# DarlingHang/st-nerf

Measured on NVIDIA H100. Metric: rays/sec, higher is better.
Workload: dtype f32 via fp16x3 split products (wgmma), f32 accumulate

## Files before the change

st-nerf_b200/csrc/mlp_tc.cu:

```cuda
#include <cuda_fp16.h>
#include <string.h>
#include <type_traits>
#include <vector>
#include "mlp_tc.cuh"
#include "resample.cuh"

namespace stnerf {

namespace {

constexpr int TILE_M = 128;
constexpr int ABLOCK = 16384;
constexpr int STAGE_BYTES = 16384;
constexpr int NTHREADS = 384;
constexpr int MATH_WG0 = 1, N_MATH_WARPS = 8;
constexpr int MAX_STAGE = 8;
constexpr int BAR_WFULL = 0, BAR_WEMPTY = 8, BAR_RAWFULL = 16, BAR_RAWEMPTY = 18;
constexpr int MISC_ROWS = 256;
constexpr int MISC_PART = MISC_ROWS + 128 * 24;
constexpr int MISC_CDF = MISC_PART + 2048;
constexpr int MISC_TOTAL = MISC_CDF + 512;

__device__ __forceinline__ uint32_t smem_u32(const void* p) { return (uint32_t)__cvta_generic_to_shared(p); }

__device__ __forceinline__ void mbar_init(uint32_t bar, uint32_t count) {
  asm volatile("mbarrier.init.shared::cta.b64 [%0], %1;" ::"r"(bar), "r"(count) : "memory");
}
__device__ __forceinline__ void mbar_arrive(uint32_t bar) {
  asm volatile("mbarrier.arrive.shared::cta.b64 _, [%0];" ::"r"(bar) : "memory");
}
__device__ __forceinline__ void mbar_arrive_if(uint32_t bar, bool pred) {
  asm volatile("{\n\t.reg .pred p;\n\tsetp.ne.b32 p, %1, 0;\n\t@p mbarrier.arrive.shared::cta.b64 _, [%0];\n\t}" ::"r"(bar), "r"((uint32_t)pred)
               : "memory");
}
__device__ __forceinline__ void mbar_expect_tx(uint32_t bar, uint32_t bytes) {
  asm volatile("mbarrier.arrive.expect_tx.shared::cta.b64 _, [%0], %1;" ::"r"(bar), "r"(bytes) : "memory");
}
__device__ __forceinline__ void mbar_wait(uint32_t bar, uint32_t parity) {
  asm volatile(
      "{\n\t.reg .pred p;\n\t.reg .u32 c;\n\t"
      "mov.u32 c, 0;\n"
      "WAIT_%=:\n\t"
      "mbarrier.try_wait.parity.shared::cta.b64 p, [%0], %1;\n\t"
      "@p bra.uni DONE_%=;\n\t"
      "add.u32 c, c, 1;\n\t"
      "setp.gt.u32 p, c, 67108864;\n\t"
      "@p trap;\n\t"
      "bra.uni WAIT_%=;\n"
      "DONE_%=:\n\t}" ::"r"(bar), "r"(parity)
      : "memory");
}
__device__ __forceinline__ void bulk_g2s(uint32_t dst, const void* src, uint32_t bytes, uint32_t bar) {
  asm volatile("cp.async.bulk.shared::cluster.global.mbarrier::complete_tx::bytes [%0], [%1], %2, [%3];" ::"r"(dst),
               "l"(src), "r"(bytes), "r"(bar)
               : "memory");
}
__device__ __forceinline__ void fence_proxy_async() { asm volatile("fence.proxy.async.shared::cta;" ::: "memory"); }
__device__ __forceinline__ void wg_bar_sync(int wg) { asm volatile("bar.sync %0, 128;" ::"r"(1 + wg) : "memory"); }

__device__ __forceinline__ void load_stage_elect(uint32_t dst, const void* src, uint32_t bytes, uint32_t bar) {
  asm volatile(
      "{\n\t.reg .pred pe;\n\t"
      "elect.sync _|pe, 0xffffffff;\n\t"
      "@pe mbarrier.arrive.expect_tx.shared::cta.b64 _, [%3], %2;\n\t"
      "@pe cp.async.bulk.shared::cluster.global.mbarrier::complete_tx::bytes [%0], [%1], %2, [%3];\n\t}" ::"r"(dst),
      "l"(src), "r"(bytes), "r"(bar)
      : "memory");
}

__device__ __forceinline__ uint64_t desc_sw128(uint32_t saddr) {
  return (uint64_t)((saddr >> 4) & 0x3FFF) | ((uint64_t)1 << 16) | ((uint64_t)(1024 >> 4) << 32) | ((uint64_t)1 << 62);
}
__device__ __forceinline__ uint64_t desc_sw64(uint32_t saddr) {
  return (uint64_t)((saddr >> 4) & 0x3FFF) | ((uint64_t)1 << 16) | ((uint64_t)(512 >> 4) << 32) | ((uint64_t)2 << 62);
}
__device__ __forceinline__ void wgmma_fence() { asm volatile("wgmma.fence.sync.aligned;" ::: "memory"); }
__device__ __forceinline__ void wgmma_commit() { asm volatile("wgmma.commit_group.sync.aligned;" ::: "memory"); }
template <int N>
__device__ __forceinline__ void wgmma_wait() { asm volatile("wgmma.wait_group.sync.aligned %0;" ::"n"(N) : "memory"); }
template <int R>
__device__ __forceinline__ void acc_fence(float (&d)[128]) {
#pragma unroll
  for (int i = 0; i < R; ++i) asm volatile("" : "+f"(d[i])::"memory");
}

__device__ __forceinline__ void wgmma_n256(float (&d)[128], uint64_t da, uint64_t db) {
  asm volatile(
      "{\n\t.reg .pred p;\n\tsetp.ne.b32 p, %130, 0;\n\t"
      "wgmma.mma_async.sync.aligned.m64n256k16.f32.f16.f16 "
      "{%0, %1, %2, %3, %4, %5, %6, %7, %8, %9, %10, %11, %12, %13, %14, %15, "
      "%16, %17, %18, %19, %20, %21, %22, %23, %24, %25, %26, %27, %28, %29, %30, %31, "
      "%32, %33, %34, %35, %36, %37, %38, %39, %40, %41, %42, %43, %44, %45, %46, %47, "
      "%48, %49, %50, %51, %52, %53, %54, %55, %56, %57, %58, %59, %60, %61, %62, %63, "
      "%64, %65, %66, %67, %68, %69, %70, %71, %72, %73, %74, %75, %76, %77, %78, %79, "
      "%80, %81, %82, %83, %84, %85, %86, %87, %88, %89, %90, %91, %92, %93, %94, %95, "
      "%96, %97, %98, %99, %100, %101, %102, %103, %104, %105, %106, %107, %108, %109, %110, %111, "
      "%112, %113, %114, %115, %116, %117, %118, %119, %120, %121, %122, %123, %124, %125, %126, %127}, "
      "%128, %129, p, 1, 1, 0, 0;\n\t}"
      : "+f"(d[0]), "+f"(d[1]), "+f"(d[2]), "+f"(d[3]), "+f"(d[4]), "+f"(d[5]), "+f"(d[6]), "+f"(d[7]),
        "+f"(d[8]), "+f"(d[9]), "+f"(d[10]), "+f"(d[11]), "+f"(d[12]), "+f"(d[13]), "+f"(d[14]), "+f"(d[15]),
        "+f"(d[16]), "+f"(d[17]), "+f"(d[18]), "+f"(d[19]), "+f"(d[20]), "+f"(d[21]), "+f"(d[22]), "+f"(d[23]),
        "+f"(d[24]), "+f"(d[25]), "+f"(d[26]), "+f"(d[27]), "+f"(d[28]), "+f"(d[29]), "+f"(d[30]), "+f"(d[31]),
        "+f"(d[32]), "+f"(d[33]), "+f"(d[34]), "+f"(d[35]), "+f"(d[36]), "+f"(d[37]), "+f"(d[38]), "+f"(d[39]),
        "+f"(d[40]), "+f"(d[41]), "+f"(d[42]), "+f"(d[43]), "+f"(d[44]), "+f"(d[45]), "+f"(d[46]), "+f"(d[47]),
        "+f"(d[48]), "+f"(d[49]), "+f"(d[50]), "+f"(d[51]), "+f"(d[52]), "+f"(d[53]), "+f"(d[54]), "+f"(d[55]),
        "+f"(d[56]), "+f"(d[57]), "+f"(d[58]), "+f"(d[59]), "+f"(d[60]), "+f"(d[61]), "+f"(d[62]), "+f"(d[63]),
        "+f"(d[64]), "+f"(d[65]), "+f"(d[66]), "+f"(d[67]), "+f"(d[68]), "+f"(d[69]), "+f"(d[70]), "+f"(d[71]),
        "+f"(d[72]), "+f"(d[73]), "+f"(d[74]), "+f"(d[75]), "+f"(d[76]), "+f"(d[77]), "+f"(d[78]), "+f"(d[79]),
        "+f"(d[80]), "+f"(d[81]), "+f"(d[82]), "+f"(d[83]), "+f"(d[84]), "+f"(d[85]), "+f"(d[86]), "+f"(d[87]),
        "+f"(d[88]), "+f"(d[89]), "+f"(d[90]), "+f"(d[91]), "+f"(d[92]), "+f"(d[93]), "+f"(d[94]), "+f"(d[95]),
        "+f"(d[96]), "+f"(d[97]), "+f"(d[98]), "+f"(d[99]), "+f"(d[100]), "+f"(d[101]), "+f"(d[102]), "+f"(d[103]),
        "+f"(d[104]), "+f"(d[105]), "+f"(d[106]), "+f"(d[107]), "+f"(d[108]), "+f"(d[109]), "+f"(d[110]), "+f"(d[111]),
        "+f"(d[112]), "+f"(d[113]), "+f"(d[114]), "+f"(d[115]), "+f"(d[116]), "+f"(d[117]), "+f"(d[118]), "+f"(d[119]),
        "+f"(d[120]), "+f"(d[121]), "+f"(d[122]), "+f"(d[123]), "+f"(d[124]), "+f"(d[125]), "+f"(d[126]), "+f"(d[127])
      : "l"(da), "l"(db), "r"(1));
}
__device__ __forceinline__ void wgmma_n128(float (&d)[128], uint64_t da, uint64_t db) {
  asm volatile(
      "{\n\t.reg .pred p;\n\tsetp.ne.b32 p, %66, 0;\n\t"
      "wgmma.mma_async.sync.aligned.m64n128k16.f32.f16.f16 "
      "{%0, %1, %2, %3, %4, %5, %6, %7, %8, %9, %10, %11, %12, %13, %14, %15, "
      "%16, %17, %18, %19, %20, %21, %22, %23, %24, %25, %26, %27, %28, %29, %30, %31, "
      "%32, %33, %34, %35, %36, %37, %38, %39, %40, %41, %42, %43, %44, %45, %46, %47, "
      "%48, %49, %50, %51, %52, %53, %54, %55, %56, %57, %58, %59, %60, %61, %62, %63}, "
      "%64, %65, p, 1, 1, 0, 0;\n\t}"
      : "+f"(d[0]), "+f"(d[1]), "+f"(d[2]), "+f"(d[3]), "+f"(d[4]), "+f"(d[5]), "+f"(d[6]), "+f"(d[7]),
        "+f"(d[8]), "+f"(d[9]), "+f"(d[10]), "+f"(d[11]), "+f"(d[12]), "+f"(d[13]), "+f"(d[14]), "+f"(d[15]),
        "+f"(d[16]), "+f"(d[17]), "+f"(d[18]), "+f"(d[19]), "+f"(d[20]), "+f"(d[21]), "+f"(d[22]), "+f"(d[23]),
        "+f"(d[24]), "+f"(d[25]), "+f"(d[26]), "+f"(d[27]), "+f"(d[28]), "+f"(d[29]), "+f"(d[30]), "+f"(d[31]),
        "+f"(d[32]), "+f"(d[33]), "+f"(d[34]), "+f"(d[35]), "+f"(d[36]), "+f"(d[37]), "+f"(d[38]), "+f"(d[39]),
        "+f"(d[40]), "+f"(d[41]), "+f"(d[42]), "+f"(d[43]), "+f"(d[44]), "+f"(d[45]), "+f"(d[46]), "+f"(d[47]),
        "+f"(d[48]), "+f"(d[49]), "+f"(d[50]), "+f"(d[51]), "+f"(d[52]), "+f"(d[53]), "+f"(d[54]), "+f"(d[55]),
        "+f"(d[56]), "+f"(d[57]), "+f"(d[58]), "+f"(d[59]), "+f"(d[60]), "+f"(d[61]), "+f"(d[62]), "+f"(d[63])
      : "l"(da), "l"(db), "r"(1));
}

template <int N>
__device__ __forceinline__ void wgmma_k16(float (&d)[128], uint64_t da, uint64_t db) {
  if (N == 256) wgmma_n256(d, da, db);
  else wgmma_n128(d, da, db);
}

__device__ __forceinline__ uint32_t pack_f16x2(float a, float b) {
  uint32_t r;
  asm("cvt.rn.satfinite.f16x2.f32 %0, %1, %2;" : "=r"(r) : "f"(b), "f"(a));
  return r;
}
__device__ __forceinline__ float2 unpack_f16x2(uint32_t p) {
  return __half22float2(*reinterpret_cast<const __half2*>(&p));
}

__host__ __device__ inline uint32_t sw128_offset(int row, int col) {
  return (uint32_t)((row >> 3) * 1024 + (row & 7) * 128 + ((((col >> 3) ^ (row & 7)) & 7) << 4) + ((col & 7) << 1));
}
__host__ __device__ inline uint32_t sw64_offset(int row, int col) {
  return (uint32_t)((row >> 3) * 512 + (row & 7) * 64 + ((((col >> 3) ^ ((row >> 1) & 3)) & 3) << 4) + ((col & 7) << 1));
}

enum { NET_SPACE = 0, NET_MOTION = 1 };

template <int NET> struct Sched;
template <> struct Sched<NET_SPACE> {
  static constexpr int N_LAYERS = 8;
  static constexpr int act_base = 0, enc_base = 8 * ABLOCK;
  static constexpr int LO_STRIDE = 4 * ABLOCK;
  static constexpr int ENC_LO_STRIDE = ABLOCK;
  static constexpr int n_stage = 3, stage_bytes = STAGE_BYTES;
  static constexpr int ring_base = 10 * ABLOCK, misc_base = ring_base + n_stage * stage_bytes, smem_total = misc_base + MISC_TOTAL;
  static_assert(smem_total <= 232448, "shared memory budget (227 KB per CTA)");
  __host__ __device__ static constexpr int n_out(int l) { return l == 7 ? 128 : 256; }
  __host__ __device__ static constexpr int act_chunks(int l) { return l == 0 ? 0 : 4; }
  __host__ __device__ static constexpr int enc_chunks(int l) { return (l == 0 || l == 4) ? 1 : 0; }
  __host__ __device__ static constexpr bool enc_first(int l) { return l == 4; }
};
template <> struct Sched<NET_MOTION> {
  static constexpr int N_LAYERS = 5;
  static constexpr int act_base = 0, enc_base = 0;
  static constexpr int LO_STRIDE = 2 * ABLOCK;
  static constexpr int ENC_LO_STRIDE = 2 * ABLOCK;
  static constexpr int n_stage = 8, stage_bytes = 8192;
  static constexpr int ring_base = 4 * ABLOCK, misc_base = ring_base + n_stage * stage_bytes, smem_total = misc_base + MISC_TOTAL;
  __host__ __device__ static constexpr int n_out(int) { return 128; }
  __host__ __device__ static constexpr int act_chunks(int l) { return l == 0 ? 0 : 2; }
  __host__ __device__ static constexpr int enc_chunks(int l) { return l == 0 ? 2 : 0; }
  __host__ __device__ static constexpr bool enc_first(int) { return false; }
};
static_assert(Sched<NET_SPACE>::n_stage <= MAX_STAGE && Sched<NET_MOTION>::n_stage <= MAX_STAGE, "barrier slots");

enum { A_HI = 0, A_LO = 1, A_HI_LO = 2 };
template <int A>
struct WStep {
  static constexpr int a = A;
  uint32_t offset;
  uint32_t sub;
};
template <int NET>
struct WSched {
  using S = Sched<NET>;
  __host__ __device__ static constexpr int n_chunks(int l) { return S::act_chunks(l) + S::enc_chunks(l); }
  __host__ __device__ static constexpr uint32_t stage_bytes(int l) { return (uint32_t)S::n_out(l) * 64; }
  __host__ __device__ static constexpr size_t layer_bytes(int l) { return (size_t)n_chunks(l) * 2  * 2  * stage_bytes(l); }
  __host__ __device__ static constexpr int chunk_at(int l, int c) {
    return S::enc_first(l) ? (c == 0 ? S::act_chunks(l) : c - 1) : c;
  }
  static constexpr bool enc_first_valid() {
    for (int l = 0; l < S::N_LAYERS; ++l)
      if (S::enc_first(l) && (S::act_chunks(l) == 0 || S::enc_chunks(l) == 0)) return false;
    return true;
  }
  static_assert(enc_first_valid(), "enc_first(l) needs activation chunks and an encoding chunk to reorder");
  template <bool LOFIRST, class C, class F>
  __device__ __forceinline__ static void for_each_step(int l, bool split, C&& chunk, F&& f) {
    const int nact = S::act_chunks(l), nch = nact + S::enc_chunks(l);
    const uint32_t bytes = stage_bytes(l);
    auto at = [&](const auto& a, int c, uint32_t sub, uint32_t lo_stage, auto op) {
      f(a, WStep<decltype(op)::value>{(2 * (2 * (uint32_t)c + sub) + lo_stage) * bytes, sub});
    };
    using HI = std::integral_constant<int, A_HI>;
    using LO = std::integral_constant<int, A_LO>;
    using HI_LO = std::integral_constant<int, A_HI_LO>;
    if (!LOFIRST || !split) {
      for (int c = 0; c < nch; ++c) {
        const auto a = chunk(chunk_at(l, c));
        for (uint32_t sub = 0; sub < 2; ++sub) {
          if (split) { at(a, c, sub, 1u, HI()); at(a, c, sub, 0u, HI_LO()); }
          else at(a, c, sub, 0u, HI());
        }
      }
    } else {
      for (int c = 0; c < nch; ++c) {
        const auto a = chunk(chunk_at(l, c));
        for (uint32_t sub = 0; sub < 2; ++sub) { at(a, c, sub, 1u, HI()); at(a, c, sub, 0u, LO()); }
      }
      for (int c = 0; c < nch; ++c) {
        const auto a = chunk(chunk_at(l, c));
        for (uint32_t sub = 0; sub < 2; ++sub) at(a, c, sub, 0u, HI());
      }
    }
  }
};

template <int NET>
__host__ __device__ constexpr size_t stream_bytes_per_tile() {
  size_t n = 0;
  for (int l = 0; l < Sched<NET>::N_LAYERS; ++l) n += WSched<NET>::layer_bytes(l);
  return n;
}

struct TcParams {
  FuseCoarse fuse;
  PointSrc src;
  const uint8_t* wstream;
  const float* aux;
  const float* cbuf;
  int exact;
  int single_last;
  int lo_first;
  float* raw;
  float* rgb_out;
// ... 145 lines not shown
        a = in4[d];
        if (lerp) {
          const float lo = d < 3 ? in4[d] : lo_t, hi = d < 3 ? in4[d] : lo_t + 1.0f;
          a = __fadd_rn(__fmul_rn(omw, lo), __fmul_rn(wgt, hi));
        }
      }
      v[8 + d] = a; v[12 + d] = 0.f;
    }
  }
  store_row_split<16>(enc, S::ENC_LO_STRIDE, row, piece * 16, v, exact);
}

template <int NET, int piece>
__device__ __forceinline__ void encode_piece(uint8_t* smem, const Pt& pt, int row, int half, bool exact, bool lerp,
                                             float (&carry)[2]) {
  if (NET == NET_SPACE) {
    if (half == 0) encode_space_piece<0, piece < 2 ? piece : 1>(smem, pt, row, exact, carry);
    else encode_space_piece<1, piece < 2 ? piece : 1>(smem, pt, row, exact, carry);
  } else {
    if (half == 0) encode_motion_piece<0, piece>(smem, pt, row, exact, lerp);
    else encode_motion_piece<1, piece>(smem, pt, row, exact, lerp);
  }
}

template <int NZ>
__device__ __noinline__ void fused_composite_loop(const TcParams& P, const float* rows, float* cdf, uint32_t bar_full, uint32_t bar_empty,
                                                  long long n_tiles, int j, int lane) {
  const FuseCoarse& F = P.fuse;
  const PointSrc& src = P.src;
  const long long n_slots = src.count ? (long long)(*src.count) : src.n_slots;
  const int n1 = 64, n2 = F.n2;
  uint32_t n = 0;
  for (long long tile = blockIdx.x; tile < n_tiles; tile += gridDim.x, ++n) {
    mbar_wait(bar_full, n & 1);
    const long long slot = tile * 2 + j;
    if (slot < n_slots) {
      const long long ray = src.hit ? (long long)src.hit[slot] : slot;
      const float* tp = src.t + ray * n1;
      const float4* rp = reinterpret_cast<const float4*>(rows) + j * 64;
      float t[2], sg[2];
#pragma unroll
      for (int s = 0; s < 2; ++s) {
        const int k = s * 32 + lane;
        const float tk = __ldg(tp + k);
        float v = rp[k].w;
        if (F.is_bkgd) {
          if (tk < F.near_plane) v = 0.0f;
        } else {
          if (tk < 0.0f) v = 0.0f;
          if (F.apply_thr && v < F.thr) v = 0.0f;
        }
        t[s] = tk;
        sg[s] = v;
      }
      const float* up = F.u ? F.u + ray * n2 : nullptr;
      const uint64_t seed = F.seed;
      const uint32_t stream = 64u + (uint32_t)F.layer;
      const unsigned long long gid = F.idmap(F.ray_base + ray);
      rs::LayerOut lo;
      rs::composite_resample_ray<2, NZ>(
          t, sg, n1, n2, F.boarder,
          [rp, lane](int s) {
            const float4 v = rp[s * 32 + lane];
            return make_float3(__fdiv_rn(1.0f, __fadd_rn(1.0f, expf(-v.x))), __fdiv_rn(1.0f, __fadd_rn(1.0f, expf(-v.y))),
                               __fdiv_rn(1.0f, __fadd_rn(1.0f, expf(-v.z))));
          },
          [up, seed, stream, gid](int jj) { return up ? up[jj] : philox_uniform(seed, stream, gid, (uint32_t)jj); },
          cdf, F.t_fine + ray * (n1 + n2), lane, lo, F.z_new ? F.z_new + ray * n2 : nullptr,
          F.z_new ? F.src_map + ray * (n1 + n2) : nullptr);
      if (F.img && lane < 5) {
        const long long rg = F.ray_base + ray;
        const float v = lane == 0 ? lo.pix[0] : lane == 1 ? lo.pix[1] : lane == 2 ? lo.pix[2] : lane == 3 ? lo.pix[3] : lo.pix[4];
        if (F.pixels) F.img[rg * 5 + lane] = v;
        else if (lane < 3) F.img[rg * 3 + lane] = v;
        else F.img[(long long)lane * F.n_total + rg] = v;
      }
    }
    __syncwarp();
    if (lane == 0) mbar_arrive(bar_empty);
  }
}

template <int NET, int N, bool LOFIRST>
__device__ __forceinline__ void mma_layer(float (&acc)[128], int l, bool sp, uint32_t sbase, uint32_t a_row, uint32_t bars,
                                          uint32_t& cnt, int lane) {
  using S = Sched<NET>;
  using W = WSched<NET>;
  constexpr uint32_t NST = S::n_stage;
#pragma unroll
  for (int i = 0; i < N / 2; ++i) acc[i] = 0.f;
  acc_fence<N / 2>(acc);
  wgmma_fence();
  const int nact = S::act_chunks(l);
  int pend = -1;
  auto release = [&](int s) {
    __syncwarp();
    mbar_arrive_if(bars + 8u * (uint32_t)(BAR_WEMPTY + s), lane == 0);
  };
  auto a_block = [&](int ch) {
    uint32_t hi, lo;
    if (ch < nact) {
      hi = sbase + S::act_base + ch * ABLOCK + a_row;
      lo = hi + S::LO_STRIDE;
    } else {
      hi = sbase + S::enc_base + (ch - nact) * ABLOCK + a_row;
      lo = hi + S::ENC_LO_STRIDE;
    }
    return make_uint2(hi, lo);
  };
  W::template for_each_step<LOFIRST>(l, sp, a_block, [&](const uint2& a, auto st) {
    const uint32_t hi = a.x + 64u * st.sub, lo = a.y + 64u * st.sub;
    const uint32_t a0 = decltype(st)::a == A_LO ? lo : hi;
    const uint32_t s = cnt % NST, n = cnt / NST;
    mbar_wait(bars + 8u * (BAR_WFULL + s), n & 1);
    const uint32_t w = sbase + S::ring_base + s * S::stage_bytes;
#pragma unroll
    for (int ks = 0; ks < 2; ++ks) wgmma_k16<N>(acc, desc_sw128(a0 + ks * 32), desc_sw64(w + ks * 32));
    if constexpr (decltype(st)::a == A_HI_LO) {
#pragma unroll
      for (int ks = 0; ks < 2; ++ks) wgmma_k16<N>(acc, desc_sw128(lo + ks * 32), desc_sw64(w + ks * 32));
    }
    wgmma_commit();
    wgmma_wait<1>();
    if (pend >= 0) release(pend);
    pend = (int)s;
    ++cnt;
  });
  wgmma_wait<0>();
  acc_fence<N / 2>(acc);
  release(pend);
}

template <int NET, int N, bool SIGMA>
__device__ __forceinline__ void epi_hidden(const float (&acc)[128], const float* __restrict__ bias, const float* __restrict__ wsig,
                                           uint8_t* smem, int r0, int cq, bool lo_too, float& sig0, float& sig1) {
  using S = Sched<NET>;
#pragma unroll
  for (int j = 0; j < N / 8; ++j) {
    const int col = 8 * j + cq;
    const float2 b = __ldg(reinterpret_cast<const float2*>(bias + col));
    const float v00 = fmaxf(acc[4 * j] + b.x, 0.f), v01 = fmaxf(acc[4 * j + 1] + b.y, 0.f);
    const float v10 = fmaxf(acc[4 * j + 2] + b.x, 0.f), v11 = fmaxf(acc[4 * j + 3] + b.y, 0.f);
    if (SIGMA) {
      const float2 w = __ldg(reinterpret_cast<const float2*>(wsig + col));
      sig0 = fmaf(v00, w.x, sig0); sig0 = fmaf(v01, w.y, sig0);
      sig1 = fmaf(v10, w.x, sig1); sig1 = fmaf(v11, w.y, sig1);
    }
    uint8_t* blk = smem + S::act_base + (col >> 6) * ABLOCK;
    const uint32_t o0 = sw128_offset(r0, col & 63), o1 = sw128_offset(r0 + 8, col & 63);
    const uint32_t h0 = pack_f16x2(v00, v01), h1 = pack_f16x2(v10, v11);
    *reinterpret_cast<uint32_t*>(blk + o0) = h0;
    *reinterpret_cast<uint32_t*>(blk + o1) = h1;
    if (lo_too) {
      const float2 f0 = unpack_f16x2(h0), f1 = unpack_f16x2(h1);
      *reinterpret_cast<uint32_t*>(blk + S::LO_STRIDE + o0) = pack_f16x2(v00 - f0.x, v01 - f0.y);
      *reinterpret_cast<uint32_t*>(blk + S::LO_STRIDE + o1) = pack_f16x2(v10 - f1.x, v11 - f1.y);
    }
  }
}

__device__ __forceinline__ float quad_sum(float v) {
  v += __shfl_xor_sync(0xffffffffu, v, 1);
  v += __shfl_xor_sync(0xffffffffu, v, 2);
  return v;
}

template <int NET, bool LOFIRST>
__global__ void __launch_bounds__(NTHREADS, 1) mlp_tc_kernel(const __grid_constant__ TcParams P) {
  using S = Sched<NET>;
  extern __shared__ __align__(1024) uint8_t smem[];
  const uint32_t sbase = smem_u32(smem);
  if ((sbase & 1023u) != 0) {
    if (threadIdx.x == 0) printf("stnerf mlp_tc: dynamic shared memory base %u is not 1024-byte aligned\n", sbase);
    __trap();
  }
  const uint32_t bars = sbase + S::misc_base;
  auto BAR = [bars](int i) { return bars + 8u * (uint32_t)i; };
  Pt* s_rows = reinterpret_cast<Pt*>(smem + S::misc_base + MISC_ROWS);
  float* s_part = reinterpret_cast<float*>(smem + S::misc_base + MISC_PART);

  const int tid = threadIdx.x, lane = tid & 31;
  const int warp = __shfl_sync(0xffffffffu, tid >> 5, 0);
  const int wgi = __shfl_sync(0xffffffffu, tid >> 7, 0);
  const bool exact = P.exact != 0;
  const bool single_last = P.single_last != 0;
  auto split = [&](int l) { return exact && !(single_last && l == S::N_LAYERS - 1); };
  const long long n_points = src_num_points(P.src);
  const long long n_tiles = (n_points + TILE_M - 1) / TILE_M;
  constexpr uint32_t NST = S::n_stage;
  if (tid == 0) {
    for (int i = 0; i < MAX_STAGE; ++i) { mbar_init(BAR(BAR_WFULL + i), 1); mbar_init(BAR(BAR_WEMPTY + i), N_MATH_WARPS); }
    for (int j = 0; j < 2; ++j) {
      mbar_init(BAR(BAR_RAWFULL + j), 4);
      mbar_init(BAR(BAR_RAWEMPTY + j), 1);
    }
    asm volatile("fence.mbarrier_init.release.cluster;" ::: "memory");
  }
  __syncthreads();

  if (warp == 0) {
    using W = WSched<NET>;
    uint32_t cnt = 0;
    for (long long tile = blockIdx.x; tile < n_tiles; tile += gridDim.x) {
      const uint8_t* layer = P.wstream;
      for (int l = 0; l < S::N_LAYERS; ++l) {
        W::template for_each_step<LOFIRST>(l, split(l), [](int) { return 0; }, [&](int, auto st) {
          const uint32_t s = cnt % NST, n = cnt / NST;
          mbar_wait(BAR(BAR_WEMPTY + s), (n & 1) ^ 1);
          load_stage_elect(sbase + S::ring_base + s * S::stage_bytes, layer + st.offset, W::stage_bytes(l), BAR(BAR_WFULL + s));
          ++cnt;
        });
        layer += W::layer_bytes(l);
      }
    }
  } else if (NET == NET_SPACE && (warp == 2 || warp == 3)) {
    if (P.fuse.on) {
      const int j = warp - 2;
      float* cdf = reinterpret_cast<float*>(smem + S::misc_base + MISC_CDF) + j * 64;
      if (P.fuse.n2 <= 128)
        fused_composite_loop<4>(P, s_part, cdf, BAR(BAR_RAWFULL + j), BAR(BAR_RAWEMPTY + j), n_tiles, j, lane);
      else
        fused_composite_loop<8>(P, s_part, cdf, BAR(BAR_RAWFULL + j), BAR(BAR_RAWEMPTY + j), n_tiles, j, lane);
    }
  } else if (wgi >= MATH_WG0) {
    const int wg = wgi - MATH_WG0;
    const int wt = tid & 127;
    const int erow = wg * 64 + (wt & 63), ehalf = wt >> 6;
    const int r0 = wg * 64 + (wt >> 5) * 16 + (lane >> 2);
    const int cq = 2 * (lane & 3);
    const uint32_t a_row = (uint32_t)wg * 8u * 1024u;
    const float* bias_all = P.aux + AUX_BIAS;
    const bool lerp = (NET == NET_MOTION) && (P.lerp_force >= 0 ? (P.lerp_force != 0) : (P.lerp_flag && *P.lerp_flag != 0));
    const bool fused = (NET == NET_SPACE) && P.fuse.on;
    uint32_t cnt = 0, tile_no = 0;
    float acc[128];
    for (long long tile = blockIdx.x; tile < n_tiles; tile += gridDim.x, ++tile_no) {
      wg_bar_sync(wg);
      const Pt cur = fetch_pt(P.src, tile * TILE_M + erow, n_points);
      if (ehalf == 0) s_rows[erow] = cur;
      float carry[2] = {0.f, 0.f};
      if (NET == NET_MOTION) {
        uint8_t* enc = smem + S::enc_base + ehalf * ABLOCK;
        for (int c = (ehalf == 0 ? 48 : 40); c < 64; c += 8) {
          const uint32_t off = sw128_offset(erow, c);
          *reinterpret_cast<uint4*>(enc + off) = make_uint4(0, 0, 0, 0);
          *reinterpret_cast<uint4*>(enc + S::ENC_LO_STRIDE + off) = make_uint4(0, 0, 0, 0);
        }
      }
      encode_piece<NET, 0>(smem, cur, erow, ehalf, exact, lerp, carry);
      encode_piece<NET, 1>(smem, cur, erow, ehalf, exact, lerp, carry);
      if (NET == NET_MOTION) encode_piece<NET, 2>(smem, cur, erow, ehalf, exact, lerp, carry);
      float sig0 = 0.f, sig1 = 0.f;
      for (int l = 0; l < S::N_LAYERS; ++l) {
        fence_proxy_async();
        wg_bar_sync(wg);
        const bool last = (l == S::N_LAYERS - 1);
        if (!last) {
          mma_layer<NET, (NET == NET_SPACE ? 256 : 128), LOFIRST>(acc, l, split(l), sbase, a_row, bars, cnt, lane);
          if (NET == NET_SPACE && l == 6)
            epi_hidden<NET, 256, true>(acc, bias_all + l * 256, P.aux + AUX_WSIG, smem, r0, cq, split(l + 1), sig0, sig1);
          else
            epi_hidden<NET, (NET == NET_SPACE ? 256 : 128), false>(acc, bias_all + l * 256, nullptr, smem, r0, cq, split(l + 1), sig0, sig1);
          continue;
        }
        mma_layer<NET, 128, LOFIRST>(acc, l, split(l), sbase, a_row, bars, cnt, lane);
        const Pt p0 = s_rows[r0], p1 = s_rows[r0 + 8];
        const float* b0 = (NET == NET_SPACE) ? (P.cbuf + (size_t)p0.cidx * 128) : bias_all + l * 256;
        const float* b1 = (NET == NET_SPACE) ? (P.cbuf + (size_t)p1.cidx * 128) : bias_all + l * 256;
        float d0[3] = {0.f, 0.f, 0.f}, d1[3] = {0.f, 0.f, 0.f};
#pragma unroll
        for (int j = 0; j < 16; ++j) {
          const int col = 8 * j + cq;
          const float2 ba = __ldg(reinterpret_cast<const float2*>(b0 + col));
          const float2 bb = __ldg(reinterpret_cast<const float2*>(b1 + col));
          const float v00 = fmaxf(acc[4 * j] + ba.x, 0.f), v01 = fmaxf(acc[4 * j + 1] + ba.y, 0.f);
          const float v10 = fmaxf(acc[4 * j + 2] + bb.x, 0.f), v11 = fmaxf(acc[4 * j + 3] + bb.y, 0.f);
#pragma unroll
          for (int o = 0; o < 3; ++o) {
            const float2 w = __ldg(reinterpret_cast<const float2*>(P.aux + AUX_WOUT + o * 128 + col));
            d0[o] = fmaf(v00, w.x, d0[o]); d0[o] = fmaf(v01, w.y, d0[o]);
            d1[o] = fmaf(v10, w.x, d1[o]); d1[o] = fmaf(v11, w.y, d1[o]);
          }
        }
#pragma unroll
        for (int o = 0; o < 3; ++o) { d0[o] = quad_sum(d0[o]) + P.aux[AUX_BOUT + o]; d1[o] = quad_sum(d1[o]) + P.aux[AUX_BOUT + o]; }
        if (NET == NET_SPACE) { sig0 = quad_sum(sig0) + P.aux[AUX_BSIG]; sig1 = quad_sum(sig1) + P.aux[AUX_BSIG]; }
        if (fused) {
          if (tile_no > 0) mbar_wait(BAR(BAR_RAWEMPTY + wg), (tile_no - 1) & 1);
          if ((lane & 3) == 0) {
            reinterpret_cast<float4*>(s_part)[r0] = make_float4(d0[0], d0[1], d0[2], sig0);
            reinterpret_cast<float4*>(s_part)[r0 + 8] = make_float4(d1[0], d1[1], d1[2], sig1);
          }
          __syncwarp();
          if (lane == 0) mbar_arrive(BAR(BAR_RAWFULL + wg));
        }
        if ((lane & 3) == 0) {
#pragma unroll
          for (int h = 0; h < 2; ++h) {
            const Pt& p = h ? p1 : p0;
            const float* o = h ? d1 : d0;
            const float sg = h ? sig1 : sig0;
            if (p.out_index < 0) continue;
            const int oi = p.out_index;
            if (NET == NET_SPACE) {
              if (P.raw) reinterpret_cast<float4*>(P.raw)[oi] = make_float4(o[0], o[1], o[2], sg);
              if (P.rgb_out) { P.rgb_out[3 * (size_t)oi] = o[0]; P.rgb_out[3 * (size_t)oi + 1] = o[1]; P.rgb_out[3 * (size_t)oi + 2] = o[2]; }
              if (P.sigma_out) P.sigma_out[oi] = sg;
            } else {
              const long long pidx = tile * TILE_M + r0 + 8 * h;
              if (P.flow_out) { P.flow_out[3 * pidx] = o[0]; P.flow_out[3 * pidx + 1] = o[1]; P.flow_out[3 * pidx + 2] = o[2]; }
              if (P.xyz_out) {
                P.xyz_out[3 * pidx] = __fadd_rn(p.x, o[0]);
                P.xyz_out[3 * pidx + 1] = __fadd_rn(p.y, o[1]);
                P.xyz_out[3 * pidx + 2] = __fadd_rn(p.z, o[2]);
              }
            }
          }
        }
      }
    }
  }
}

constexpr int HB_SLOTS = 8;
__global__ void __launch_bounds__(128) head_bias_kernel(PointSrc src, const float* __restrict__ w_tail ,
                                                        const float* __restrict__ b1, int use_time,
                                                        float* __restrict__ cbuf) {
  __shared__ float s_enc[HB_SLOTS][48];
  const long long n_slots = src.count ? (long long)(*src.count) : src.n_slots;
  const int nk = PE_DIR + (use_time ? PE_TIME : 0);
  const int tid = threadIdx.x;
  float w[48];
#pragma unroll
  for (int k = 0; k < 48; ++k) w[k] = (k < nk) ? __ldg(w_tail + k * 128 + tid) : 0.f;
  const float bias = __ldg(b1 + tid);
  for (long long s0 = (long long)blockIdx.x * HB_SLOTS; s0 < n_slots; s0 += (long long)gridDim.x * HB_SLOTS) {
    __syncthreads();
    for (int e = tid; e < HB_SLOTS * 48; e += 128) {
      const int sl = e / 48, j = e - sl * 48;
      const long long slot = s0 + sl;
      float v = 0.f;
      if (slot < n_slots && j < nk) {
        float d[3], tm;
        if (src.mode == SRC_EXPLICIT) {
          d[0] = src.dirs[3 * slot]; d[1] = src.dirs[3 * slot + 1]; d[2] = src.dirs[3 * slot + 2];
          tm = src.times ? src.times[slot * src.time_stride] : 0.f;
        } else {
          const long long ray = src.hit ? (long long)src.hit[slot] : slot;
// ... 344 lines not shown
```

Baseline: 721,000.

## Keep fp16 low-part activations in registers and feed them via register-A wgmma

For the space network, the low-order fp16 residual of each hidden activation is kept in a 64-entry register array and passed to wgmma through the register-sourced A-operand form, instead of being written to and read back from shared memory. This frees four activation blocks of shared memory, which are used to deepen the weight ring from 3 to 7 stages. setmaxnreg moves registers from the producer warpgroup to the math warpgroups to hold the extra state. Risks include register pressure or spills, and the unrolled selection over the register index adds branching around each wgmma.

New measurement: 749,900 (median of 6 runs). 4.0% higher.

```diff
diff --git a/st-nerf_b200/csrc/mlp_tc.cu b/st-nerf_b200/csrc/mlp_tc.cu
--- a/st-nerf_b200/csrc/mlp_tc.cu
+++ b/st-nerf_b200/csrc/mlp_tc.cu
@@ -15,6 +15,8 @@
 constexpr int NTHREADS = 384;
 constexpr int MATH_WG0 = 1, N_MATH_WARPS = 8;
 constexpr int MAX_STAGE = 8;
+constexpr int REGS_WG0 = 56, REGS_MATH = 224;
+static_assert(128 * REGS_WG0 + 256 * REGS_MATH <= 384 * 168, "register file");
 constexpr int BAR_WFULL = 0, BAR_WEMPTY = 8, BAR_RAWFULL = 16, BAR_RAWEMPTY = 18;
 constexpr int MISC_ROWS = 256;
 constexpr int MISC_PART = MISC_ROWS + 128 * 24;
@@ -56,6 +58,10 @@
                : "memory");
 }
 __device__ __forceinline__ void fence_proxy_async() { asm volatile("fence.proxy.async.shared::cta;" ::: "memory"); }
+template <int R>
+__device__ __forceinline__ void setmaxnreg_dec() { asm volatile("setmaxnreg.dec.sync.aligned.u32 %0;" ::"n"(R)); }
+template <int R>
+__device__ __forceinline__ void setmaxnreg_inc() { asm volatile("setmaxnreg.inc.sync.aligned.u32 %0;" ::"n"(R)); }
 __device__ __forceinline__ void wg_bar_sync(int wg) { asm volatile("bar.sync %0, 128;" ::"r"(1 + wg) : "memory"); }
 
 __device__ __forceinline__ void load_stage_elect(uint32_t dst, const void* src, uint32_t bytes, uint32_t bar) {
@@ -84,55 +90,58 @@
   for (int i = 0; i < R; ++i) asm volatile("" : "+f"(d[i])::"memory");
 }
 
+#define WGMMA_D_LO "%0, %1, %2, %3, %4, %5, %6, %7, %8, %9, %10, %11, %12, %13, %14, %15, %16, %17, %18, %19, %20, %21, %22, %23, %24, %25, %26, %27, %28, %29, %30, %31, %32, %33, %34, %35, %36, %37, %38, %39, %40, %41, %42, %43, %44, %45, %46, %47, %48, %49, %50, %51, %52, %53, %54, %55, %56, %57, %58, %59, %60, %61, %62, %63"
+#define WGMMA_D_HI "%64, %65, %66, %67, %68, %69, %70, %71, %72, %73, %74, %75, %76, %77, %78, %79, %80, %81, %82, %83, %84, %85, %86, %87, %88, %89, %90, %91, %92, %93, %94, %95, %96, %97, %98, %99, %100, %101, %102, %103, %104, %105, %106, %107, %108, %109, %110, %111, %112, %113, %114, %115, %116, %117, %118, %119, %120, %121, %122, %123, %124, %125, %126, %127"
+#define WGMMA_OPS_LO(d) \
+    "+f"(d[0]), "+f"(d[1]), "+f"(d[2]), "+f"(d[3]), "+f"(d[4]), "+f"(d[5]), "+f"(d[6]), "+f"(d[7]), \
+    "+f"(d[8]), "+f"(d[9]), "+f"(d[10]), "+f"(d[11]), "+f"(d[12]), "+f"(d[13]), "+f"(d[14]), "+f"(d[15]), \
+    "+f"(d[16]), "+f"(d[17]), "+f"(d[18]), "+f"(d[19]), "+f"(d[20]), "+f"(d[21]), "+f"(d[22]), "+f"(d[23]), \
+    "+f"(d[24]), "+f"(d[25]), "+f"(d[26]), "+f"(d[27]), "+f"(d[28]), "+f"(d[29]), "+f"(d[30]), "+f"(d[31]), \
+    "+f"(d[32]), "+f"(d[33]), "+f"(d[34]), "+f"(d[35]), "+f"(d[36]), "+f"(d[37]), "+f"(d[38]), "+f"(d[39]), \
+    "+f"(d[40]), "+f"(d[41]), "+f"(d[42]), "+f"(d[43]), "+f"(d[44]), "+f"(d[45]), "+f"(d[46]), "+f"(d[47]), \
+    "+f"(d[48]), "+f"(d[49]), "+f"(d[50]), "+f"(d[51]), "+f"(d[52]), "+f"(d[53]), "+f"(d[54]), "+f"(d[55]), \
+    "+f"(d[56]), "+f"(d[57]), "+f"(d[58]), "+f"(d[59]), "+f"(d[60]), "+f"(d[61]), "+f"(d[62]), "+f"(d[63])
+#define WGMMA_OPS_HI(d) \
+    "+f"(d[64]), "+f"(d[65]), "+f"(d[66]), "+f"(d[67]), "+f"(d[68]), "+f"(d[69]), "+f"(d[70]), "+f"(d[71]), \
+    "+f"(d[72]), "+f"(d[73]), "+f"(d[74]), "+f"(d[75]), "+f"(d[76]), "+f"(d[77]), "+f"(d[78]), "+f"(d[79]), \
+    "+f"(d[80]), "+f"(d[81]), "+f"(d[82]), "+f"(d[83]), "+f"(d[84]), "+f"(d[85]), "+f"(d[86]), "+f"(d[87]), \
+    "+f"(d[88]), "+f"(d[89]), "+f"(d[90]), "+f"(d[91]), "+f"(d[92]), "+f"(d[93]), "+f"(d[94]), "+f"(d[95]), \
+    "+f"(d[96]), "+f"(d[97]), "+f"(d[98]), "+f"(d[99]), "+f"(d[100]), "+f"(d[101]), "+f"(d[102]), "+f"(d[103]), \
+    "+f"(d[104]), "+f"(d[105]), "+f"(d[106]), "+f"(d[107]), "+f"(d[108]), "+f"(d[109]), "+f"(d[110]), "+f"(d[111]), \
+    "+f"(d[112]), "+f"(d[113]), "+f"(d[114]), "+f"(d[115]), "+f"(d[116]), "+f"(d[117]), "+f"(d[118]), "+f"(d[119]), \
+    "+f"(d[120]), "+f"(d[121]), "+f"(d[122]), "+f"(d[123]), "+f"(d[124]), "+f"(d[125]), "+f"(d[126]), "+f"(d[127])
+
 __device__ __forceinline__ void wgmma_n256(float (&d)[128], uint64_t da, uint64_t db) {
   asm volatile(
       "{\n\t.reg .pred p;\n\tsetp.ne.b32 p, %130, 0;\n\t"
       "wgmma.mma_async.sync.aligned.m64n256k16.f32.f16.f16 "
-      "{%0, %1, %2, %3, %4, %5, %6, %7, %8, %9, %10, %11, %12, %13, %14, %15, "
-      "%16, %17, %18, %19, %20, %21, %22, %23, %24, %25, %26, %27, %28, %29, %30, %31, "
-      "%32, %33, %34, %35, %36, %37, %38, %39, %40, %41, %42, %43, %44, %45, %46, %47, "
-      "%48, %49, %50, %51, %52, %53, %54, %55, %56, %57, %58, %59, %60, %61, %62, %63, "
-      "%64, %65, %66, %67, %68, %69, %70, %71, %72, %73, %74, %75, %76, %77, %78, %79, "
-      "%80, %81, %82, %83, %84, %85, %86, %87, %88, %89, %90, %91, %92, %93, %94, %95, "
-      "%96, %97, %98, %99, %100, %101, %102, %103, %104, %105, %106, %107, %108, %109, %110, %111, "
-      "%112, %113, %114, %115, %116, %117, %118, %119, %120, %121, %122, %123, %124, %125, %126, %127}, "
-      "%128, %129, p, 1, 1, 0, 0;\n\t}"
-      : "+f"(d[0]), "+f"(d[1]), "+f"(d[2]), "+f"(d[3]), "+f"(d[4]), "+f"(d[5]), "+f"(d[6]), "+f"(d[7]),
-        "+f"(d[8]), "+f"(d[9]), "+f"(d[10]), "+f"(d[11]), "+f"(d[12]), "+f"(d[13]), "+f"(d[14]), "+f"(d[15]),
-        "+f"(d[16]), "+f"(d[17]), "+f"(d[18]), "+f"(d[19]), "+f"(d[20]), "+f"(d[21]), "+f"(d[22]), "+f"(d[23]),
-        "+f"(d[24]), "+f"(d[25]), "+f"(d[26]), "+f"(d[27]), "+f"(d[28]), "+f"(d[29]), "+f"(d[30]), "+f"(d[31]),
-        "+f"(d[32]), "+f"(d[33]), "+f"(d[34]), "+f"(d[35]), "+f"(d[36]), "+f"(d[37]), "+f"(d[38]), "+f"(d[39]),
-        "+f"(d[40]), "+f"(d[41]), "+f"(d[42]), "+f"(d[43]), "+f"(d[44]), "+f"(d[45]), "+f"(d[46]), "+f"(d[47]),
-        "+f"(d[48]), "+f"(d[49]), "+f"(d[50]), "+f"(d[51]), "+f"(d[52]), "+f"(d[53]), "+f"(d[54]), "+f"(d[55]),
-        "+f"(d[56]), "+f"(d[57]), "+f"(d[58]), "+f"(d[59]), "+f"(d[60]), "+f"(d[61]), "+f"(d[62]), "+f"(d[63]),
-        "+f"(d[64]), "+f"(d[65]), "+f"(d[66]), "+f"(d[67]), "+f"(d[68]), "+f"(d[69]), "+f"(d[70]), "+f"(d[71]),
-        "+f"(d[72]), "+f"(d[73]), "+f"(d[74]), "+f"(d[75]), "+f"(d[76]), "+f"(d[77]), "+f"(d[78]), "+f"(d[79]),
-        "+f"(d[80]), "+f"(d[81]), "+f"(d[82]), "+f"(d[83]), "+f"(d[84]), "+f"(d[85]), "+f"(d[86]), "+f"(d[87]),
-        "+f"(d[88]), "+f"(d[89]), "+f"(d[90]), "+f"(d[91]), "+f"(d[92]), "+f"(d[93]), "+f"(d[94]), "+f"(d[95]),
-        "+f"(d[96]), "+f"(d[97]), "+f"(d[98]), "+f"(d[99]), "+f"(d[100]), "+f"(d[101]), "+f"(d[102]), "+f"(d[103]),
-        "+f"(d[104]), "+f"(d[105]), "+f"(d[106]), "+f"(d[107]), "+f"(d[108]), "+f"(d[109]), "+f"(d[110]), "+f"(d[111]),
-        "+f"(d[112]), "+f"(d[113]), "+f"(d[114]), "+f"(d[115]), "+f"(d[116]), "+f"(d[117]), "+f"(d[118]), "+f"(d[119]),
-        "+f"(d[120]), "+f"(d[121]), "+f"(d[122]), "+f"(d[123]), "+f"(d[124]), "+f"(d[125]), "+f"(d[126]), "+f"(d[127])
+      "{" WGMMA_D_LO ", " WGMMA_D_HI "}, %128, %129, p, 1, 1, 0, 0;\n\t}"
+      : WGMMA_OPS_LO(d), WGMMA_OPS_HI(d)
       : "l"(da), "l"(db), "r"(1));
 }
 __device__ __forceinline__ void wgmma_n128(float (&d)[128], uint64_t da, uint64_t db) {
   asm volatile(
       "{\n\t.reg .pred p;\n\tsetp.ne.b32 p, %66, 0;\n\t"
       "wgmma.mma_async.sync.aligned.m64n128k16.f32.f16.f16 "
-      "{%0, %1, %2, %3, %4, %5, %6, %7, %8, %9, %10, %11, %12, %13, %14, %15, "
-      "%16, %17, %18, %19, %20, %21, %22, %23, %24, %25, %26, %27, %28, %29, %30, %31, "
-      "%32, %33, %34, %35, %36, %37, %38, %39, %40, %41, %42, %43, %44, %45, %46, %47, "
-      "%48, %49, %50, %51, %52, %53, %54, %55, %56, %57, %58, %59, %60, %61, %62, %63}, "
-      "%64, %65, p, 1, 1, 0, 0;\n\t}"
-      : "+f"(d[0]), "+f"(d[1]), "+f"(d[2]), "+f"(d[3]), "+f"(d[4]), "+f"(d[5]), "+f"(d[6]), "+f"(d[7]),
-        "+f"(d[8]), "+f"(d[9]), "+f"(d[10]), "+f"(d[11]), "+f"(d[12]), "+f"(d[13]), "+f"(d[14]), "+f"(d[15]),
-        "+f"(d[16]), "+f"(d[17]), "+f"(d[18]), "+f"(d[19]), "+f"(d[20]), "+f"(d[21]), "+f"(d[22]), "+f"(d[23]),
-        "+f"(d[24]), "+f"(d[25]), "+f"(d[26]), "+f"(d[27]), "+f"(d[28]), "+f"(d[29]), "+f"(d[30]), "+f"(d[31]),
-        "+f"(d[32]), "+f"(d[33]), "+f"(d[34]), "+f"(d[35]), "+f"(d[36]), "+f"(d[37]), "+f"(d[38]), "+f"(d[39]),
-        "+f"(d[40]), "+f"(d[41]), "+f"(d[42]), "+f"(d[43]), "+f"(d[44]), "+f"(d[45]), "+f"(d[46]), "+f"(d[47]),
-        "+f"(d[48]), "+f"(d[49]), "+f"(d[50]), "+f"(d[51]), "+f"(d[52]), "+f"(d[53]), "+f"(d[54]), "+f"(d[55]),
-        "+f"(d[56]), "+f"(d[57]), "+f"(d[58]), "+f"(d[59]), "+f"(d[60]), "+f"(d[61]), "+f"(d[62]), "+f"(d[63])
+      "{" WGMMA_D_LO "}, %64, %65, p, 1, 1, 0, 0;\n\t}"
+      : WGMMA_OPS_LO(d)
       : "l"(da), "l"(db), "r"(1));
+}
+__device__ __forceinline__ void wgmma_n256_rs(float (&d)[128], const uint32_t* a, uint64_t db) {
+  asm volatile(
+      "{\n\t.reg .pred p;\n\tsetp.ne.b32 p, %133, 0;\n\t"
+      "wgmma.mma_async.sync.aligned.m64n256k16.f32.f16.f16 "
+      "{" WGMMA_D_LO ", " WGMMA_D_HI "}, {%128, %129, %130, %131}, %132, p, 1, 1, 0;\n\t}"
+      : WGMMA_OPS_LO(d), WGMMA_OPS_HI(d)
+      : "r"(a[0]), "r"(a[1]), "r"(a[2]), "r"(a[3]), "l"(db), "r"(1));
+}
+__device__ __forceinline__ void wgmma_n128_rs(float (&d)[128], const uint32_t* a, uint64_t db) {
+  asm volatile(
+      "{\n\t.reg .pred p;\n\tsetp.ne.b32 p, %69, 0;\n\t"
+      "wgmma.mma_async.sync.aligned.m64n128k16.f32.f16.f16 "
+      "{" WGMMA_D_LO "}, {%64, %65, %66, %67}, %68, p, 1, 1, 0;\n\t}"
+      : WGMMA_OPS_LO(d)
+      : "r"(a[0]), "r"(a[1]), "r"(a[2]), "r"(a[3]), "l"(db), "r"(1));
 }
 
 template <int N>
@@ -140,6 +149,11 @@
   if (N == 256) wgmma_n256(d, da, db);
   else wgmma_n128(d, da, db);
 }
+template <int N>
+__device__ __forceinline__ void wgmma_k16_rs(float (&d)[128], const uint32_t* a, uint64_t db) {
+  if (N == 256) wgmma_n256_rs(d, a, db);
+  else wgmma_n128_rs(d, a, db);
+}
 
 __device__ __forceinline__ uint32_t pack_f16x2(float a, float b) {
   uint32_t r;
@@ -162,11 +176,11 @@
 template <int NET> struct Sched;
 template <> struct Sched<NET_SPACE> {
   static constexpr int N_LAYERS = 8;
-  static constexpr int act_base = 0, enc_base = 8 * ABLOCK;
-  static constexpr int LO_STRIDE = 4 * ABLOCK;
+  static constexpr bool lo_in_regs = true;
+  static constexpr int act_base = 0, enc_base = 4 * ABLOCK;
   static constexpr int ENC_LO_STRIDE = ABLOCK;
-  static constexpr int n_stage = 3, stage_bytes = STAGE_BYTES;
-  static constexpr int ring_base = 10 * ABLOCK, misc_base = ring_base + n_stage * stage_bytes, smem_total = misc_base + MISC_TOTAL;
+  static constexpr int n_stage = 7, stage_bytes = STAGE_BYTES;
+  static constexpr int ring_base = 6 * ABLOCK, misc_base = ring_base + n_stage * stage_bytes, smem_total = misc_base + MISC_TOTAL;
   static_assert(smem_total <= 232448, "shared memory budget (227 KB per CTA)");
   __host__ __device__ static constexpr int n_out(int l) { return l == 7 ? 128 : 256; }
   __host__ __device__ static constexpr int act_chunks(int l) { return l == 0 ? 0 : 4; }
@@ -175,6 +189,7 @@
 };
 template <> struct Sched<NET_MOTION> {
   static constexpr int N_LAYERS = 5;
+  static constexpr bool lo_in_regs = false;
   static constexpr int act_base = 0, enc_base = 0;
   static constexpr int LO_STRIDE = 2 * ABLOCK;
   static constexpr int ENC_LO_STRIDE = 2 * ABLOCK;
@@ -486,8 +501,8 @@
 }
 
 template <int NET, int N, bool LOFIRST>
-__device__ __forceinline__ void mma_layer(float (&acc)[128], int l, bool sp, uint32_t sbase, uint32_t a_row, uint32_t bars,
-                                          uint32_t& cnt, int lane) {
+__device__ __forceinline__ void mma_layer(float (&acc)[128], const uint32_t (&alo)[64], int l, bool sp, uint32_t sbase,
+                                          uint32_t a_row, uint32_t bars, uint32_t& cnt, int lane) {
   using S = Sched<NET>;
   using W = WSched<NET>;
   constexpr uint32_t NST = S::n_stage;
@@ -502,27 +517,43 @@
     mbar_arrive_if(bars + 8u * (uint32_t)(BAR_WEMPTY + s), lane == 0);
   };
   auto a_block = [&](int ch) {
-    uint32_t hi, lo;
+    uint32_t hi, lo = 0;
+    int z = -1;
     if (ch < nact) {
       hi = sbase + S::act_base + ch * ABLOCK + a_row;
-      lo = hi + S::LO_STRIDE;
+      if constexpr (S::lo_in_regs) z = ch;
+      else lo = hi + S::LO_STRIDE;
     } else {
       hi = sbase + S::enc_base + (ch - nact) * ABLOCK + a_row;
       lo = hi + S::ENC_LO_STRIDE;
     }
-    return make_uint2(hi, lo);
+    return make_int3((int)hi, (int)lo, z);
   };
-  W::template for_each_step<LOFIRST>(l, sp, a_block, [&](const uint2& a, auto st) {
-    const uint32_t hi = a.x + 64u * st.sub, lo = a.y + 64u * st.sub;
-    const uint32_t a0 = decltype(st)::a == A_LO ? lo : hi;
+  W::template for_each_step<LOFIRST>(l, sp, a_block, [&](const int3& a, auto st) {
+    const uint32_t hi = (uint32_t)a.x + 64u * st.sub, lo = (uint32_t)a.y + 64u * st.sub;
     const uint32_t s = cnt % NST, n = cnt / NST;
     mbar_wait(bars + 8u * (BAR_WFULL + s), n & 1);
     const uint32_t w = sbase + S::ring_base + s * S::stage_bytes;
-#pragma unroll
-    for (int ks = 0; ks < 2; ++ks) wgmma_k16<N>(acc, desc_sw128(a0 + ks * 32), desc_sw64(w + ks * 32));
-    if constexpr (decltype(st)::a == A_HI_LO) {
-#pragma unroll
-      for (int ks = 0; ks < 2; ++ks) wgmma_k16<N>(acc, desc_sw128(lo + ks * 32), desc_sw64(w + ks * 32));
+    auto mma_lo = [&]() {
+      if (S::lo_in_regs && a.z >= 0) {
+        const int q = 2 * a.z + (int)st.sub;
+#pragma unroll
+        for (int i = 0; i < 8; ++i)
+          if (q == i) {
+#pragma unroll
+            for (int ks = 0; ks < 2; ++ks) wgmma_k16_rs<N>(acc, &alo[8 * i + 4 * ks], desc_sw64(w + ks * 32));
+          }
+      } else {
+#pragma unroll
+        for (int ks = 0; ks < 2; ++ks) wgmma_k16<N>(acc, desc_sw128(lo + ks * 32), desc_sw64(w + ks * 32));
+      }
+    };
+    if constexpr (decltype(st)::a == A_LO) {
+      mma_lo();
+    } else {
+#pragma unroll
+      for (int ks = 0; ks < 2; ++ks) wgmma_k16<N>(acc, desc_sw128(hi + ks * 32), desc_sw64(w + ks * 32));
+      if constexpr (decltype(st)::a == A_HI_LO) mma_lo();
     }
     wgmma_commit();
     wgmma_wait<1>();
@@ -537,7 +568,8 @@
 
 template <int NET, int N, bool SIGMA>
 __device__ __forceinline__ void epi_hidden(const float (&acc)[128], const float* __restrict__ bias, const float* __restrict__ wsig,
-                                           uint8_t* smem, int r0, int cq, bool lo_too, float& sig0, float& sig1) {
+                                           uint8_t* smem, int r0, int cq, bool lo_too, float& sig0, float& sig1,
+                                           uint32_t (&alo)[64]) {
   using S = Sched<NET>;
 #pragma unroll
   for (int j = 0; j < N / 8; ++j) {
@@ -555,10 +587,14 @@
     const uint32_t h0 = pack_f16x2(v00, v01), h1 = pack_f16x2(v10, v11);
     *reinterpret_cast<uint32_t*>(blk + o0) = h0;
     *reinterpret_cast<uint32_t*>(blk + o1) = h1;
-    if (lo_too) {
-      const float2 f0 = unpack_f16x2(h0), f1 = unpack_f16x2(h1);
-      *reinterpret_cast<uint32_t*>(blk + S::LO_STRIDE + o0) = pack_f16x2(v00 - f0.x, v01 - f0.y);
-      *reinterpret_cast<uint32_t*>(blk + S::LO_STRIDE + o1) = pack_f16x2(v10 - f1.x, v11 - f1.y);
+    const float2 f0 = unpack_f16x2(h0), f1 = unpack_f16x2(h1);
+    const uint32_t l0 = pack_f16x2(v00 - f0.x, v01 - f0.y), l1 = pack_f16x2(v10 - f1.x, v11 - f1.y);
+    if constexpr (S::lo_in_regs) {
+      alo[2 * j] = l0;
+      alo[2 * j + 1] = l1;
+    } else if (lo_too) {
+      *reinterpret_cast<uint32_t*>(blk + S::LO_STRIDE + o0) = l0;
+      *reinterpret_cast<uint32_t*>(blk + S::LO_STRIDE + o1) = l1;
     }
   }
 }
@@ -602,31 +638,35 @@
   }
   __syncthreads();
 
-  if (warp == 0) {
-    using W = WSched<NET>;
-    uint32_t cnt = 0;
-    for (long long tile = blockIdx.x; tile < n_tiles; tile += gridDim.x) {
-      const uint8_t* layer = P.wstream;
-      for (int l = 0; l < S::N_LAYERS; ++l) {
-        W::template for_each_step<LOFIRST>(l, split(l), [](int) { return 0; }, [&](int, auto st) {
-          const uint32_t s = cnt % NST, n = cnt / NST;
-          mbar_wait(BAR(BAR_WEMPTY + s), (n & 1) ^ 1);
-          load_stage_elect(sbase + S::ring_base + s * S::stage_bytes, layer + st.offset, W::stage_bytes(l), BAR(BAR_WFULL + s));
-          ++cnt;
-        });
-        layer += W::layer_bytes(l);
-      }
-    }
-  } else if (NET == NET_SPACE && (warp == 2 || warp == 3)) {
-    if (P.fuse.on) {
-      const int j = warp - 2;
-      float* cdf = reinterpret_cast<float*>(smem + S::misc_base + MISC_CDF) + j * 64;
-      if (P.fuse.n2 <= 128)
-        fused_composite_loop<4>(P, s_part, cdf, BAR(BAR_RAWFULL + j), BAR(BAR_RAWEMPTY + j), n_tiles, j, lane);
-      else
-        fused_composite_loop<8>(P, s_part, cdf, BAR(BAR_RAWFULL + j), BAR(BAR_RAWEMPTY + j), n_tiles, j, lane);
-    }
-  } else if (wgi >= MATH_WG0) {
+  if (wgi < MATH_WG0) {
+    if constexpr (S::lo_in_regs) setmaxnreg_dec<REGS_WG0>();
+    if (warp == 0) {
+      using W = WSched<NET>;
+      uint32_t cnt = 0;
+      for (long long tile = blockIdx.x; tile < n_tiles; tile += gridDim.x) {
+        const uint8_t* layer = P.wstream;
+        for (int l = 0; l < S::N_LAYERS; ++l) {
+          W::template for_each_step<LOFIRST>(l, split(l), [](int) { return 0; }, [&](int, auto st) {
+            const uint32_t s = cnt % NST, n = cnt / NST;
+            mbar_wait(BAR(BAR_WEMPTY + s), (n & 1) ^ 1);
+            load_stage_elect(sbase + S::ring_base + s * S::stage_bytes, layer + st.offset, W::stage_bytes(l), BAR(BAR_WFULL + s));
+            ++cnt;
+          });
+          layer += W::layer_bytes(l);
+        }
+      }
+    } else if (NET == NET_SPACE && (warp == 2 || warp == 3)) {
+      if (P.fuse.on) {
+        const int j = warp - 2;
+        float* cdf = reinterpret_cast<float*>(smem + S::misc_base + MISC_CDF) + j * 64;
+        if (P.fuse.n2 <= 128)
+          fused_composite_loop<4>(P, s_part, cdf, BAR(BAR_RAWFULL + j), BAR(BAR_RAWEMPTY + j), n_tiles, j, lane);
+        else
+          fused_composite_loop<8>(P, s_part, cdf, BAR(BAR_RAWFULL + j), BAR(BAR_RAWEMPTY + j), n_tiles, j, lane);
+      }
+    }
+  } else {
+    if constexpr (S::lo_in_regs) setmaxnreg_inc<REGS_MATH>();
     const int wg = wgi - MATH_WG0;
     const int wt = tid & 127;
     const int erow = wg * 64 + (wt & 63), ehalf = wt >> 6;
@@ -638,6 +678,9 @@
     const bool fused = (NET == NET_SPACE) && P.fuse.on;
     uint32_t cnt = 0, tile_no = 0;
     float acc[128];
+    uint32_t alo[64];
+#pragma unroll
+    for (int i = 0; i < 64; ++i) alo[i] = 0u;
     for (long long tile = blockIdx.x; tile < n_tiles; tile += gridDim.x, ++tile_no) {
       wg_bar_sync(wg);
       const Pt cur = fetch_pt(P.src, tile * TILE_M + erow, n_points);
@@ -660,14 +703,15 @@
         wg_bar_sync(wg);
         const bool last = (l == S::N_LAYERS - 1);
         if (!last) {
-          mma_layer<NET, (NET == NET_SPACE ? 256 : 128), LOFIRST>(acc, l, split(l), sbase, a_row, bars, cnt, lane);
+          mma_layer<NET, (NET == NET_SPACE ? 256 : 128), LOFIRST>(acc, alo, l, split(l), sbase, a_row, bars, cnt, lane);
           if (NET == NET_SPACE && l == 6)
-            epi_hidden<NET, 256, true>(acc, bias_all + l * 256, P.aux + AUX_WSIG, smem, r0, cq, split(l + 1), sig0, sig1);
+            epi_hidden<NET, 256, true>(acc, bias_all + l * 256, P.aux + AUX_WSIG, smem, r0, cq, split(l + 1), sig0, sig1, alo);
           else
-            epi_hidden<NET, (NET == NET_SPACE ? 256 : 128), false>(acc, bias_all + l * 256, nullptr, smem, r0, cq, split(l + 1), sig0, sig1);
+            epi_hidden<NET, (NET == NET_SPACE ? 256 : 128), false>(acc, bias_all + l * 256, nullptr, smem, r0, cq, split(l + 1), sig0,
+                                                                  sig1, alo);
           continue;
         }
-        mma_layer<NET, 128, LOFIRST>(acc, l, split(l), sbase, a_row, bars, cnt, lane);
+        mma_layer<NET, 128, LOFIRST>(acc, alo, l, split(l), sbase, a_row, bars, cnt, lane);
         const Pt p0 = s_rows[r0], p1 = s_rows[r0 + 8];
         const float* b0 = (NET == NET_SPACE) ? (P.cbuf + (size_t)p0.cidx * 128) : bias_all + l * 256;
         const float* b1 = (NET == NET_SPACE) ? (P.cbuf + (size_t)p1.cidx * 128) : bias_all + l * 256;
```
